# tikroeger/OF_DIS

Measured on AMD Instinct MI355X. Metric: frames/sec at 1024×436 op-point-2 (INT), higher is better.
Workload: dtype f32

## Files before the change

### of_dis_amd/csrc/ofdis_prep.hip

```cpp
#include <algorithm>
#include <type_traits>

#include "ofdis_kernels.h"
#include "ofdis_tvmath.h"

namespace ofdis {
namespace OFDIS_KNS {

typedef unsigned u32x2 __attribute__((ext_vector_type(2)));
typedef unsigned u32x4 __attribute__((ext_vector_type(4)));

struct WarpTaps {
  float dx, dy, m;
  int o11, o12, o21, o22;
};
__device__ __forceinline__ WarpTaps warp_taps(int tmp_w, int pad, int w, int h, int i, int j, float fx, float fy) {
  WarpTaps t;
  const float xx = i + fx;
  const float yy = j + fy;
  const int x = (int)floorf(xx), y = (int)floorf(yy);
  t.dx = xx - (float)x;
  t.dy = yy - (float)y;
  t.m = (xx >= 0 && xx <= (float)(w - 1) && yy >= 0 && yy <= (float)(h - 1)) ? 1.0f : 0.0f;
  const int x1 = clampi(x, 0, w - 1) + pad, x2 = clampi(x + 1, 0, w - 1) + pad;
  const int y1 = (clampi(y, 0, h - 1) + pad) * tmp_w, y2 = (clampi(y + 1, 0, h - 1) + pad) * tmp_w;
  t.o11 = y1 + x1; t.o12 = y1 + x2; t.o21 = y2 + x1; t.o22 = y2 + x2;
  return t;
}
__device__ __forceinline__ float warp_mix(float s11, float s12, float s21, float s22, float dx, float dy) {
  return s11 * (1.0f - dx) * (1.0f - dy) + s12 * dx * (1.0f - dy) + s21 * (1.0f - dx) * dy + s22 * dx * dy;
}

template <int FORM>
__device__ __forceinline__ float v5r(float m2, float m1, float s0, float p1, float p2) {
  if (FORM == 0) return (D5_C0 + D5_C1 + D5_C2) * s0 + D5_C3 * p1 + D5_C4 * p2;
  if (FORM == 1) return (D5_C0 + D5_C1) * m1 + D5_C2 * s0 + D5_C3 * p1 + D5_C4 * p2;
  if (FORM == 3) return D5_C0 * m2 + D5_C1 * m1 + D5_C2 * s0 + (D5_C3 + D5_C4) * p1;
  if (FORM == 4) return D5_C0 * m2 + D5_C1 * m1 + (D5_C2 + D5_C3 + D5_C4) * s0;
  return D5_C0 * m2 + D5_C1 * m1 + D5_C2 * s0 + D5_C3 * p1 + D5_C4 * p2;
}
template <typename F>
__device__ __forceinline__ void vform(int j, int h, F&& f) {
  if (j == 0) f(std::integral_constant<int, 0>());
  else if (j == 1) f(std::integral_constant<int, 1>());
  else if (j == h - 2) f(std::integral_constant<int, 3>());
  else if (j == h - 1) f(std::integral_constant<int, 4>());
  else f(std::integral_constant<int, 2>());
}
__device__ __forceinline__ float h5r(float m2, float m1, float s0, float p1, float p2) {
  return D5_C0 * m2 + D5_C1 * m1 + D5_C2 * s0 + D5_C3 * p1 + D5_C4 * p2;
}

constexpr int PREP_KD = 4;
constexpr int PREP_KW = 8;

template <int WPF>
struct PrepLds {
  static constexpr int ROW = 64 * WPF + 32;
  static constexpr int nq(int lpf, int K) { return lpf + K - 1; }
  static constexpr int STD = (WPF >= 2 ? nq(64 * WPF, PREP_KD) * PREP_KD : 4 * nq(16, PREP_KD) * PREP_KD) * 8 + 8;
  static constexpr int STW = (WPF >= 2 ? nq(64 * WPF, PREP_KW) * PREP_KW : 4 * nq(16, PREP_KW) * PREP_KW) * 2 + 2;
  static constexpr int TOTAL = 3 * ROW + STD + STW;
};

template <int WPF>
__device__ __forceinline__ void prep_sync() {
  if (WPF == 1) __builtin_amdgcn_wave_barrier();
  else asm volatile("s_waitcnt lgkmcnt(0)\n\ts_barrier" ::: "memory");
}

template <int WPF, bool DENS>
__global__ __launch_bounds__(64 * WPF) void tv_prep_kernel(const PrepArgs a, const int lpf_shift, const int nbands) {
  constexpr int C = 1;
  using L = PrepLds<WPF>;
  __shared__ __attribute__((aligned(16))) float lds[L::TOTAL];
  const int lane = threadIdx.x;
  const int w = a.t.w, h = a.t.h, S = a.S;
  const int lpf = WPF >= 2 ? 64 * WPF : (1 << lpf_shift);
  const int fpw = WPF >= 2 ? 1 : (64 >> lpf_shift);
  const int unit = blockIdx.x;
  const int fg = unit / nbands, band = unit - fg * nbands;
  const int fl = WPF >= 2 ? 0 : lane >> lpf_shift, li = WPF >= 2 ? lane : lane & (lpf - 1);
  int frame = fg * fpw + fl;
  const bool fok = frame < a.t.nframes;
  if (!fok) frame = a.t.nframes - 1;
  const int yb0 = band * a.band_rows, yb1 = min(h, yb0 + a.band_rows);
  if (yb0 >= h) return;
  const int r_begin = max(yb0 - 4, 0), r_s0end = min(yb1 + 4, h);
  const int y1lo = max(yb0 - 2, 0), y1hi = min(yb1 + 2, h);
  const int r_last = yb1 + 3;

  const int seg = lpf * C + 8;
  float* const rowA = lds + fl * seg;
  float* const rowX = lds + L::ROW + fl * seg;
  float* const rowZ = lds + 2 * L::ROW + fl * seg;
  const int nqd = L::nq(lpf, PREP_KD), nqw = L::nq(lpf, PREP_KW);
  float* const stD = lds + 3 * L::ROW;
  float* const stW = stD + L::STD;
  float* const stDf = stD + fl * nqd * PREP_KD * 8;
  float* const stWf = stW + fl * nqw * PREP_KW * 2;
  const int e0 = 2 + li * C;

  int xc[C];
  const int rw = S * w;
#pragma unroll
  for (int k = 0; k < C; ++k) xc[k] = min(li * C + k, w - 1);
  const int sg0 = (fg * fpw) / S;
  const size_t strip_recs = (size_t)rw * h;
  const int nstrips = (a.t.nframes + S - 1) / S;
  const unsigned span = (unsigned)min(nstrips - sg0, fpw + 1);
  const __amdgpu_buffer_rsrc_t rsD = __builtin_amdgcn_make_buffer_rsrc(
      (void*)(a.d8 + (size_t)sg0 * strip_recs * 8), 0, (int)(span * strip_recs * 32), 0x00020000);
  const __amdgpu_buffer_rsrc_t rsW = __builtin_amdgcn_make_buffer_rsrc(
      (void*)(a.wrec + (size_t)sg0 * strip_recs * 2), 0, (int)(span * strip_recs * 8), 0x00020000);
  const int f0 = fg * fpw, nfr = min(fpw, a.t.nframes - f0), flc = frame - f0;
  const int plane = a.tmp_w * a.tmp_h;
  const __amdgpu_buffer_rsrc_t rsF = __builtin_amdgcn_make_buffer_rsrc(
      (void*)(a.flow + (size_t)f0 * w * h * 2), 0, nfr * w * h * 8, 0x00020000);
  const __amdgpu_buffer_rsrc_t rsI = __builtin_amdgcn_make_buffer_rsrc(
      (void*)(a.im1 + (size_t)f0 * plane), 0, nfr * plane * 4, 0x00020000);
  const __amdgpu_buffer_rsrc_t rsT = __builtin_amdgcn_make_buffer_rsrc(
      (void*)(a.im2 + (size_t)f0 * plane), 0, nfr * plane * 4, 0x00020000);
  int voF[C], voI[C];
  const int voT = flc * plane * 4;
#pragma unroll
  for (int k = 0; k < C; ++k) {
    voF[k] = (flc * w * h + xc[k]) * 8;
    voI[k] = (flc * plane + a.pad * a.tmp_w + a.pad + xc[k]) * 4;
  }
  auto asf = [](unsigned u) { return __builtin_bit_cast(float, u); };
  const int nopw = a.dens_nopw, noph = a.dens_noph, nop = nopw * noph;
  __amdgpu_buffer_rsrc_t rsPW = rsF, rsP = rsF;
  int voPW[2] = {0, 0}, voP[2] = {0, 0};
  bool okx[2] = {false, false};
  if constexpr (DENS) {
    static_assert(C == 1, "one column per lane");
    rsPW = __builtin_amdgcn_make_buffer_rsrc((void*)(a.dens_pweight + (size_t)f0 * nop * 64), 0, nfr * nop * 256, 0x00020000);
    rsP = __builtin_amdgcn_make_buffer_rsrc((void*)(a.dens_p + (size_t)f0 * nop * 2), 0, nfr * nop * 8, 0x00020000);
    const int xs = xc[0] - a.dens_offw + 4, bx = xs >> 2, tx = xs & 3;
#pragma unroll
    for (int col = 0; col < 2; ++col) {
      const int gx = bx - 1 + col;
      okx[col] = (gx >= 0) & (gx < nopw);
      const int gxc = clampi(gx, 0, nopw - 1);
      voPW[col] = (flc * nop * 64 + gxc * 8 + (col ? tx : 4 + tx)) * 4;
      voP[col] = (flc * nop * 2 + gxc * 2) * 4;
    }
  }

  auto flush = [&](auto kc, auto bytes_c, const float* st, const __amdgpu_buffer_rsrc_t& rs, int nq, int y0, int yend) {
    constexpr int K = decltype(kc)::value, RB = decltype(bytes_c)::value;
    constexpr int PB = RB >= 16 ? 16 : 8;
    constexpr int PPR = RB / PB;
    constexpr int RUN = K * PPR;
    const bool full = y0 + K <= yend;
    const int nqv = S == 1 ? w : w + K - 1;
    const int iters = (nqv * RUN + 64 * WPF - 1) / (64 * WPF);
    for (int f = 0; f < fpw; ++f) {
      const int fr = f0 + f;
      if (fr >= a.t.nframes) break;
      const int sgf = fr / S, fsf = fr - sgf * S;
      const int dbase = (fsf * w + y0) % rw;
      const int base = ((sgf - sg0) * rw * h + y0) * RB;
      const float* stf = st + f * nq * K * (RB / 4);
      for (int it = 0; it < iters; ++it) {
        const int e = min(lane + it * 64 * WPF, nqv * RUN);
        const int q = e / RUN, lo = e % RUN;
        int d = dbase + q;
        d -= d >= rw ? rw : 0;
        const int k = lo / PPR, x = q - k;
        const bool ok = (q < nqv) & ((S == 1) | ((x >= 0) & (x < w))) & (full | (y0 + k < yend));
        const int byte = ok ? base + d * (h * RB) + lo * PB : 0x7ffffff0;
        if constexpr (PB == 16) {
          const u32x4 v = *reinterpret_cast<const u32x4*>(stf + e * 4);
          __builtin_amdgcn_raw_buffer_store_b128(v, rs, byte, 0, 0);
        } else {
          const u32x2 v = *reinterpret_cast<const u32x2*>(stf + e * 2);
          __builtin_amdgcn_raw_buffer_store_b64(v, rs, byte, 0, 0);
        }
      }
    }
  };
  const int col_entry = li < w ? 2 + li : lpf + 4;
  const int pad_entry = li == 0 ? 0 : (li == w - 1 ? 2 + w : lpf + 6);
  auto put_row = [&](float* row, const float (&v)[C]) {
    static_assert(C == 1, "one column per lane");
    row[col_entry] = v[0];
    row[pad_entry] = v[0];
    row[pad_entry + 1] = v[0];
  };
  auto stq = [&](int x, int k) { int q = x + k; if (S == 1 && q >= w) q -= w; return q; };

  float A[5][C], Z[5][C], IX[5][C], IY[5][C];
  float ixy1[C], ixy2[C], iyz1[C], iyz2[C];
  unsigned mbits[C];
#pragma unroll
  for (int k = 0; k < C; ++k) {
#pragma unroll
    for (int q = 0; q < 5; ++q) A[q][k] = Z[q][k] = IX[q][k] = IY[q][k] = 0.0f;
    ixy1[k] = ixy2[k] = iyz1[k] = iyz2[k] = 0.0f;
    mbits[k] = 0;
  }

  struct Pend {
    float fx, fy, i1;
  };
  Pend nxt[C], cur[C];
  WarpTaps tp[C];
  float t11[C], t12[C], t21[C], t22[C];
  unsigned lf0[C], lf1[C], li1[C];
  unsigned dpw[4], dp0[4], dp1[4];
  auto request_row = [&](int row) {
    const int rr = min(row, h - 1);
    if constexpr (DENS) {
      const int ys = rr - a.dens_offh + 4, by = ys >> 2, ty = ys & 3;
#pragma unroll
      for (int rsel = 0; rsel < 2; ++rsel) {
        const int gyc = clampi(by - 1 + rsel, 0, noph - 1), ky = rsel ? ty : 4 + ty;
        const int soPW = (gyc * 8 + ky) * nopw * 32, soP = gyc * nopw * 8;
#pragma unroll
        for (int col = 0; col < 2; ++col) {
          dpw[2 * col + rsel] = __builtin_amdgcn_raw_buffer_load_b32(rsPW, voPW[col], soPW, 0);
          const auto pp = __builtin_amdgcn_raw_buffer_load_b64(rsP, voP[col], soP, 0);
          const unsigned q0 = pp[0], q1 = pp[1];
          dp0[2 * col + rsel] = q0; dp1[2 * col + rsel] = q1;
        }
      }
    }
#pragma unroll
    for (int k = 0; k < C; ++k) {
      if constexpr (!DENS) {
        const auto f = __builtin_amdgcn_raw_buffer_load_b64(rsF, voF[k], rr * w * 8, 0);
        const unsigned q0 = f[0], q1 = f[1];
        lf0[k] = q0; lf1[k] = q1;
      }
      li1[k] = __builtin_amdgcn_raw_buffer_load_b32(rsI, voI[k], rr * a.tmp_w * 4, 0);
    }
  };
  auto take_row = [&](int row) {
#pragma unroll
    for (int k = 0; k < C; ++k) {
      if constexpr (DENS) {
        const int ys = min(row, h - 1) - a.dens_offh + 4, by = ys >> 2;
        const bool okr[2] = {by >= 1 && by - 1 < noph, by < noph};
        float we = 0.0f, fu = 0.0f, fv = 0.0f;
#pragma unroll
        for (int c = 0; c < 4; ++c) {
          const bool ok = okx[c >> 1] & okr[c & 1];
          const float absw = div_rn(1.0f, fmaxf(2.0f, asf(dpw[c])));
          const float nwe = we + absw, nfu = fu + asf(dp0[c]) * absw, nfv = fv + asf(dp1[c]) * absw;
          we = ok ? nwe : we;
          fu = ok ? nfu : fu;
          fv = ok ? nfv : fv;
        }
        if (we > 0) {
          if constexpr (kFusedContract) {
            const float rwe = rcp_refined(we);
            fu *= rwe;
            fv *= rwe;
          } else {
            fu /= we;
            fv /= we;
          }
        }
        nxt[k] = Pend{fu, fv, asf(li1[k])};
      } else {
        nxt[k] = Pend{asf(lf0[k]), asf(lf1[k]), asf(li1[k])};
      }
    }
  };
  auto request_taps = [&](int row) {
    const int rr = min(row, h - 1);
    WarpTaps t[C];
#pragma unroll
    for (int k = 0; k < C; ++k) t[k] = warp_taps(a.tmp_w, a.pad, w, h, xc[k], rr, nxt[k].fx, nxt[k].fy);
#pragma unroll
    for (int k = 0; k < C; ++k) {
      t11[k] = asf(__builtin_amdgcn_raw_buffer_load_b32(rsT, voT + t[k].o11 * 4, 0, 0));
      t12[k] = asf(__builtin_amdgcn_raw_buffer_load_b32(rsT, voT + t[k].o12 * 4, 0, 0));
      t21[k] = asf(__builtin_amdgcn_raw_buffer_load_b32(rsT, voT + t[k].o21 * 4, 0, 0));
      t22[k] = asf(__builtin_amdgcn_raw_buffer_load_b32(rsT, voT + t[k].o22 * 4, 0, 0));
      tp[k] = t[k];
    }
  };
  request_row(r_begin);
  take_row(r_begin);
  request_taps(r_begin);
#pragma unroll
  for (int k = 0; k < C; ++k) cur[k] = nxt[k];
  request_row(r_begin + 1);

  for (int rb = r_begin; rb <= r_last; rb += 5) {
#pragma unroll
    for (int u = 0; u < 5; ++u) {
      const int r = rb + u;
      if (r > r_last) break;
      if (r < r_s0end) {
        float fx[C], fy[C];
#pragma unroll
        for (int k = 0; k < C; ++k) {
          fx[k] = cur[k].fx; fy[k] = cur[k].fy;
          const float i2 = warp_mix(t11[k], t12[k], t21[k], t22[k], tp[k].dx, tp[k].dy);
          mbits[k] = (mbits[k] << 1) | (tp[k].m != 0.0f ? 1u : 0u);
          A[u][k] = 0.5f * (i2 + cur[k].i1);
          Z[u][k] = i2 - cur[k].i1;
        }
        take_row(r + 1);
        request_taps(r + 1);
#pragma unroll
        for (int k = 0; k < C; ++k) cur[k] = nxt[k];
        request_row(r + 2);
        put_row(rowA, A[u]);
        if (r >= yb0 && r < yb1) {
          const int kk = (r - yb0) % PREP_KW;
          float* dst = li < w ? stWf + (stq(xc[0], kk) * PREP_KW + kk) * 2 : stW + (L::STW - 2);
          *reinterpret_cast<float2*>(dst) = make_float2(fx[0], fy[0]);
        }
        prep_sync<WPF>();
        {
          const float al0 = rowA[e0 - 2], al1 = rowA[e0 - 1], ar0 = rowA[e0 + C], ar1 = rowA[e0 + C + 1];
          if constexpr (C == 1) {
            IX[u][0] = h5r(al0, al1, A[u][0], ar0, ar1);
          } else {
            IX[u][0] = h5r(al0, al1, A[u][0], A[u][1], ar0);
            IX[u][1] = h5r(al1, A[u][0], A[u][1], ar0, ar1);
            if (li * 2 + 1 >= w) IX[u][1] = IX[u][0];
          }
        }
        if (r >= yb0 && r < yb1 && ((r - yb0) % PREP_KW == PREP_KW - 1 || r == yb1 - 1)) {
          const int y0 = r - (r - yb0) % PREP_KW;
          flush(std::integral_constant<int, PREP_KW>(), std::integral_constant<int, 8>(), stW, rsW, nqw, y0, yb1);
        }
      } else {
#pragma unroll
        for (int k = 0; k < C; ++k) mbits[k] <<= 1;
      }
      const int y1 = r - 2;
      float ixyn[C], iyzn[C];
#pragma unroll
      for (int k = 0; k < C; ++k) ixyn[k] = iyzn[k] = 0.0f;
      if (y1 >= y1lo && y1 < y1hi) {
        vform(y1, h, [&](auto form) {
          constexpr int F = decltype(form)::value;
#pragma unroll
          for (int k = 0; k < C; ++k) {
            IY[(u + 3) % 5][k] = v5r<F>(A[(u + 1) % 5][k], A[(u + 2) % 5][k], A[(u + 3) % 5][k], A[(u + 4) % 5][k], A[u][k]);
            ixyn[k] = v5r<F>(IX[(u + 1) % 5][k], IX[(u + 2) % 5][k], IX[(u + 3) % 5][k], IX[(u + 4) % 5][k], IX[u][k]);
            iyzn[k] = v5r<F>(Z[(u + 1) % 5][k], Z[(u + 2) % 5][k], Z[(u + 3) % 5][k], Z[(u + 4) % 5][k], Z[u][k]);
          }
        });
      }
      const int y2 = r - 4;
      if (y2 >= yb0 && y2 < yb1) {
        const int o = (u + 1) % 5;
        put_row(rowX, IX[o]);
        put_row(rowZ, Z[o]);
        prep_sync<WPF>();
        float ixx[C], ixz[C], iyy[C];
        {
          const float xl0 = rowX[e0 - 2], xl1 = rowX[e0 - 1], xr0 = rowX[e0 + C], xr1 = rowX[e0 + C + 1];
          const float zl0 = rowZ[e0 - 2], zl1 = rowZ[e0 - 1], zr0 = rowZ[e0 + C], zr1 = rowZ[e0 + C + 1];
          if constexpr (C == 1) {
            ixx[0] = h5r(xl0, xl1, IX[o][0], xr0, xr1);
            ixz[0] = h5r(zl0, zl1, Z[o][0], zr0, zr1);
          } else {
            ixx[0] = h5r(xl0, xl1, IX[o][0], IX[o][1], xr0);
            ixx[1] = h5r(xl1, IX[o][0], IX[o][1], xr0, xr1);
            ixz[0] = h5r(zl0, zl1, Z[o][0], Z[o][1], zr0);
            ixz[1] = h5r(zl1, Z[o][0], Z[o][1], zr0, zr1);
          }
        }
        vform(y2, h, [&](auto form) {
          constexpr int F = decltype(form)::value;
#pragma unroll
          for (int k = 0; k < C; ++k)
            iyy[k] = v5r<F>(IY[(u + 4) % 5][k], IY[u][k], IY[(u + 1) % 5][k], IY[(u + 2) % 5][k], IY[(u + 3) % 5][k]);
        });
        const int kk = (y2 - yb0) % PREP_KD;
        {
          constexpr int k = 0;
          const bool on = (mbits[k] >> 4) & 1u;
          float* dst = li < w ? stDf + (stq(xc[k], kk) * PREP_KD + kk) * 8 : stD + (L::STD - 8);
          *reinterpret_cast<float4*>(dst) =
              on ? make_float4(IX[o][k], Z[o][k], ixx[k], ixz[k]) : make_float4(0.0f, 0.0f, 0.0f, 0.0f);
          *reinterpret_cast<float4*>(dst + 4) =
              on ? make_float4(IY[o][k], ixy2[k], iyz2[k], iyy[k]) : make_float4(0.0f, 0.0f, 0.0f, 0.0f);
        }
        prep_sync<WPF>();
        if (kk == PREP_KD - 1 || y2 == yb1 - 1) {
          flush(std::integral_constant<int, PREP_KD>(), std::integral_constant<int, 32>(), stD, rsD, nqd, y2 - kk, yb1);
          prep_sync<WPF>();
        }
      }
      else {
        prep_sync<WPF>();
      }
#pragma unroll
      for (int k = 0; k < C; ++k) { ixy2[k] = ixy1[k]; iyz2[k] = iyz1[k]; ixy1[k] = ixyn[k]; iyz1[k] = iyzn[k]; }
    }
  }
}

bool tv_prep_supported(const TvGeom& t) { return t.noc == 1 && t.w >= 16 && t.w <= 256 && t.h >= 4 && t.h <= 256; }
bool tv_prep_densifies(const LevelGeom& g) { return densify_quad_geometry(g); }

hipError_t launch_tv_prep(const PrepArgs& a_in, hipStream_t s) {
  if (!tv_prep_supported(a_in.t) || a_in.S < 1) return hipErrorInvalidValue;
  PrepArgs a = a_in;
  const int w = a.t.w, h = a.t.h;
  const int lpf_shift = w > 64 ? 7 : (w > 32 ? 6 : (w > 16 ? 5 : 4));
  const int fpw = w > 64 ? 1 : (64 >> lpf_shift);
  const int fgroups = (a.t.nframes + fpw - 1) / fpw;
  int nbands;
  if (a.band_rows > 0) {
    a.band_rows = std::max(2, (a.band_rows + 1) & ~1);
  } else {
    nbands = std::max(1, std::min((2048 + fgroups - 1) / fgroups, (h + 1) / 2));
    a.band_rows = ((h + nbands - 1) / nbands + 1) & ~1;
    if (a.band_rows > PREP_KW) a.band_rows = ((a.band_rows + PREP_KW - 1) / PREP_KW) * PREP_KW;
  }
  nbands = (h + a.band_rows - 1) / a.band_rows;
  const long long units = (long long)fgroups * nbands;
  if (a.dens_p && (!a.dens_pweight || a.dens_offw < 0 || a.dens_offw > 3 || a.dens_offh < 0 || a.dens_offh > 3 || a.dens_nopw < 1 ||
                   a.dens_noph < 1))
    return hipErrorInvalidValue;
  with_constant<1, 2, 3, 4>((w + 63) / 64, [&](auto WPF) {
    with_constant<false, true>(a.dens_p != nullptr, [&](auto DENS) {
      hipLaunchKernelGGL((tv_prep_kernel<decltype(WPF)::value, decltype(DENS)::value>), dim3((unsigned)units),
                         dim3(64 * decltype(WPF)::value), 0, s, a, lpf_shift, nbands);
    });
  });
  return hipGetLastError();
}

}
}
```

Before: 1.633 million.

## Carry densified patch displacements across rows in registers instead of reloading

```diff
diff --git a/of_dis_amd/csrc/ofdis_prep.hip b/of_dis_amd/csrc/ofdis_prep.hip
--- a/of_dis_amd/csrc/ofdis_prep.hip
+++ b/of_dis_amd/csrc/ofdis_prep.hip
@@ -147,6 +147,7 @@
       voP[col] = (flc * nop * 2 + gxc * 2) * 4;
     }
   }
+  const int voPstep = voP[1] - voP[0];
 
   auto flush = [&](auto kc, auto bytes_c, const float* st, const __amdgpu_buffer_rsrc_t& rs, int nq, int y0, int yend) {
     constexpr int K = decltype(kc)::value, RB = decltype(bytes_c)::value;
@@ -210,10 +211,19 @@
   float t11[C], t12[C], t21[C], t22[C];
   unsigned lf0[C], lf1[C], li1[C];
   unsigned dpw[4], dp0[4], dp1[4];
-  auto request_row = [&](int row) {
+  unsigned la0[2], la1[2];
+  unsigned ld0 = 0, ld1 = 0;
+  auto grid_ys = [&](int row) { return min(row, h - 1) - a.dens_offh + 4; };
+  auto load_disp = [&](int vo, int so, unsigned& d0, unsigned& d1) {
+    const auto pp = __builtin_amdgcn_raw_buffer_load_b64(rsP, vo, so, 0);
+    const unsigned q0 = pp[0], q1 = pp[1];
+    d0 = q0; d1 = q1;
+  };
+  auto request_row = [&](int row, auto first) {
+    constexpr bool FIRST = decltype(first)::value;
     const int rr = min(row, h - 1);
     if constexpr (DENS) {
-      const int ys = rr - a.dens_offh + 4, by = ys >> 2, ty = ys & 3;
+      const int ys = grid_ys(row), by = ys >> 2, ty = ys & 3;
 #pragma unroll
       for (int rsel = 0; rsel < 2; ++rsel) {
         const int gyc = clampi(by - 1 + rsel, 0, noph - 1), ky = rsel ? ty : 4 + ty;
@@ -221,10 +231,15 @@
 #pragma unroll
         for (int col = 0; col < 2; ++col) {
           dpw[2 * col + rsel] = __builtin_amdgcn_raw_buffer_load_b32(rsPW, voPW[col], soPW, 0);
-          const auto pp = __builtin_amdgcn_raw_buffer_load_b64(rsP, voP[col], soP, 0);
-          const unsigned q0 = pp[0], q1 = pp[1];
-          dp0[2 * col + rsel] = q0; dp1[2 * col + rsel] = q1;
-        }
+          if constexpr (FIRST) load_disp(voP[col], soP, dp0[2 * col + rsel], dp1[2 * col + rsel]);
+        }
+      }
+      const int soLA = clampi(by + 1, 0, noph - 1) * nopw * 8;
+      if constexpr (FIRST) {
+#pragma unroll
+        for (int col = 0; col < 2; ++col) load_disp(voP[col], soLA, la0[col], la1[col]);
+      } else {
+        load_disp(voP[0] + (ty & 1) * voPstep, soLA, ld0, ld1);
       }
     }
 #pragma unroll
@@ -237,11 +252,24 @@
       li1[k] = __builtin_amdgcn_raw_buffer_load_b32(rsI, voI[k], rr * a.tmp_w * 4, 0);
     }
   };
-  auto take_row = [&](int row) {
+  auto take_row = [&](int row, auto first) {
+    if constexpr (DENS && !decltype(first)::value) {
+      const int ys = grid_ys(row);
+      const bool rot = (ys >> 2) != (grid_ys(row - 1) >> 2), odd = (ys & 1) != 0;
+#pragma unroll
+      for (int col = 0; col < 2; ++col) {
+        dp0[2 * col] = rot ? dp0[2 * col + 1] : dp0[2 * col];
+        dp1[2 * col] = rot ? dp1[2 * col + 1] : dp1[2 * col];
+        dp0[2 * col + 1] = rot ? la0[col] : dp0[2 * col + 1];
+        dp1[2 * col + 1] = rot ? la1[col] : dp1[2 * col + 1];
+        la0[col] = odd == (col == 1) ? ld0 : la0[col];
+        la1[col] = odd == (col == 1) ? ld1 : la1[col];
+      }
+    }
 #pragma unroll
     for (int k = 0; k < C; ++k) {
       if constexpr (DENS) {
-        const int ys = min(row, h - 1) - a.dens_offh + 4, by = ys >> 2;
+        const int ys = grid_ys(row), by = ys >> 2;
         const bool okr[2] = {by >= 1 && by - 1 < noph, by < noph};
         float we = 0.0f, fu = 0.0f, fv = 0.0f;
 #pragma unroll
@@ -283,12 +311,12 @@
       tp[k] = t[k];
     }
   };
-  request_row(r_begin);
-  take_row(r_begin);
+  request_row(r_begin, std::true_type());
+  take_row(r_begin, std::true_type());
   request_taps(r_begin);
 #pragma unroll
   for (int k = 0; k < C; ++k) cur[k] = nxt[k];
-  request_row(r_begin + 1);
+  request_row(r_begin + 1, std::false_type());
 
   for (int rb = r_begin; rb <= r_last; rb += 5) {
 #pragma unroll
@@ -305,11 +333,11 @@
           A[u][k] = 0.5f * (i2 + cur[k].i1);
           Z[u][k] = i2 - cur[k].i1;
         }
-        take_row(r + 1);
+        take_row(r + 1, std::false_type());
         request_taps(r + 1);
 #pragma unroll
         for (int k = 0; k < C; ++k) cur[k] = nxt[k];
-        request_row(r + 2);
+        request_row(r + 2, std::false_type());
         put_row(rowA, A[u]);
         if (r >= yb0 && r < yb1) {
           const int kk = (r - yb0) % PREP_KW;
```

Result: no change. 1.630 million (-0.2%).
